# pananananas/MVD

Hardware: AMD Instinct MI355X
Metric: UNet forward-passes/sec @512x512 SD2.1+MV adapter (higher is better)
Workload: dtype bf16; 1 GPU; cfg4: configs[3]/[4]: 8 objects x 4 target views per GPU (32 pairs), camera FiLM + cross-view adapter; pairs_per_gpu=32, global_pairs=32, latent=64x64x4, image=512x512, forward=cold, hip_graph=False, q2_statistics=replica-local, parallelism=dp1 (pairs sharded by object), weights=synthetic seeded, SD2.1 shapes (865.9M UNet x2 + 99.2M adapter + 19.1M camera), encoder_weights=distinct

## Files before the change

### include/mvd_hip.h

```cpp
#ifndef MVD_HIP_H
#define MVD_HIP_H
#include <stddef.h>
#include <stdint.h>

#ifdef __cplusplus
extern "C" {
#endif

#define MVD_MAX_LEVELS 4

typedef struct {
  int in_channels;
  int out_channels;
  int num_levels;
  int block_out_channels[MVD_MAX_LEVELS];
  int num_heads[MVD_MAX_LEVELS];
  int layers_per_block;
  int cross_attention_dim;
  int norm_num_groups;
  float norm_eps;
  int cam_output_dim;
  int cam_hidden_dim;
  int simple_cam_encoder;
  float cam_modulation_strength;
// ... 5 lines not shown

int mvd_engine_create(const mvd_config_t* cfg, mvd_engine_t** out);
int mvd_engine_destroy(mvd_engine_t* e);

int mvd_engine_set_weight(mvd_engine_t* e, int set, const char* slot, const void* ptr, int64_t numel, int dtype);
int mvd_engine_clear_weights(mvd_engine_t* e, int set);

int64_t mvd_engine_workspace_bytes(mvd_engine_t* e, int batch, int height, int width, int text_len, int ref_batch);
int64_t mvd_engine_refcache_bytes(mvd_engine_t* e, int ref_batch, int height, int width, int keep_features);
int mvd_engine_bind_workspace(mvd_engine_t* e, void* ws, int64_t ws_bytes, void* refcache, int64_t refcache_bytes);

enum {
  MVD_USE_CAMERA = 1,
  MVD_USE_IMAGE = 2,
  MVD_REUSE_REF = 4,
  MVD_KEEP_FEATURES = 8
};

typedef struct {
  int batch;
  int height, width;
  int text_len;
  const float* sample;
  const float* timesteps;
  const float* text;
  const float* source_camera;
  const float* target_camera;
  int cam_rows;
  int cam_batch;
  const float* fourier_proj;
  const float* source_latents;
  const float* encoder_text;
  int ref_batch;
  int flags;
  float* out;
} mvd_forward_args_t;

int mvd_unet_forward(mvd_engine_t* e, const mvd_forward_args_t* args, void* stream);

int64_t mvd_engine_reference_pixels(mvd_engine_t* e, int height, int width);
int mvd_engine_reference_encode(mvd_engine_t* e, const mvd_forward_args_t* args, float* local_stats, void* stream);
int mvd_engine_reference_finish(mvd_engine_t* e, const float* mean_k, void* stream);

int mvd_engine_set_graph(mvd_engine_t* e, int enable);

int mvd_engine_share_encoder_weights(mvd_engine_t* e, int enable);

int mvd_engine_set_profiling(mvd_engine_t* e, int enable);
int mvd_engine_profile_summary(mvd_engine_t* e, int cap, int* cls, int* launches, double* ms, double* flops, double* bytes);
int mvd_engine_profile_shapes(mvd_engine_t* e, char* buf_host, int cap);

int mvd_engine_num_features(mvd_engine_t* e);
int mvd_engine_feature_shape(mvd_engine_t* e, int idx, int* channels, int* height, int* width);
// ... 192 lines not shown
```

### mvd_amd/_lib.py

```python
from __future__ import annotations

import ctypes as C
import enum
import os

HERE = os.path.dirname(os.path.abspath(__file__))
LIB_PATH = os.environ.get("MVD_HIP_LIB") or os.path.join(HERE, "libmvd_hip.so")

MVD_MAX_LEVELS = 4
MVD_USE_CAMERA, MVD_USE_IMAGE, MVD_REUSE_REF, MVD_KEEP_FEATURES = 1, 2, 4, 8


class MvdError(RuntimeError):
    pass


class DebugFlag(enum.IntFlag):
    NO_SM_LN_FOLD = 1
    SM_NO_SPLITK = 2
    NO_SM = 4
    NO_SPLIT_KV = 8
    ONE_STREAM = 16
    SINGLE_STREAM_POLICY = 32
    SIDE_DEFAULT_PRIORITY = 64
    NO_XS = 128
# ... 55 lines not shown
        ("fourier_proj", C.c_void_p), ("source_latents", C.c_void_p), ("encoder_text", C.c_void_p),
        ("ref_batch", C.c_int), ("flags", C.c_int), ("out", C.c_void_p),
    ]


_SIGS = {
    "mvd_last_error": (C.c_char_p, []),
    "mvd_engine_create": (C.c_int, [C.POINTER(mvd_config_t), C.POINTER(C.c_void_p)]),
    "mvd_engine_destroy": (C.c_int, [C.c_void_p]),
    "mvd_engine_set_weight": (C.c_int, [C.c_void_p, C.c_int, C.c_char_p, C.c_void_p, C.c_int64, C.c_int]),
    "mvd_engine_clear_weights": (C.c_int, [C.c_void_p, C.c_int]),
    "mvd_engine_workspace_bytes": (C.c_int64, [C.c_void_p, C.c_int, C.c_int, C.c_int, C.c_int, C.c_int]),
    "mvd_engine_refcache_bytes": (C.c_int64, [C.c_void_p, C.c_int, C.c_int, C.c_int, C.c_int]),
    "mvd_engine_bind_workspace": (C.c_int, [C.c_void_p, C.c_void_p, C.c_int64, C.c_void_p, C.c_int64]),
    "mvd_unet_forward": (C.c_int, [C.c_void_p, C.POINTER(mvd_forward_args_t), C.c_void_p]),
    "mvd_engine_set_profiling": (C.c_int, [C.c_void_p, C.c_int]),
    "mvd_engine_profile_summary": (C.c_int, [C.c_void_p, C.c_int, C.POINTER(C.c_int), C.POINTER(C.c_int),
                                             C.POINTER(C.c_double), C.POINTER(C.c_double), C.POINTER(C.c_double)]),
    "mvd_engine_profile_shapes": (C.c_int, [C.c_void_p, C.c_char_p, C.c_int]),
    "mvd_engine_set_graph": (C.c_int, [C.c_void_p, C.c_int]),
    "mvd_engine_reference_pixels": (C.c_int64, [C.c_void_p, C.c_int, C.c_int]),
    "mvd_engine_reference_encode": (C.c_int, [C.c_void_p, C.POINTER(mvd_forward_args_t), C.c_void_p, C.c_void_p]),
    "mvd_engine_reference_finish": (C.c_int, [C.c_void_p, C.c_void_p, C.c_void_p]),
    "mvd_engine_share_encoder_weights": (C.c_int, [C.c_void_p, C.c_int]),
    "mvd_engine_num_features": (C.c_int, [C.c_void_p]),
    "mvd_engine_feature_shape": (C.c_int, [C.c_void_p, C.c_int, C.POINTER(C.c_int), C.POINTER(C.c_int), C.POINTER(C.c_int)]),
    "mvd_engine_get_feature": (C.c_int, [C.c_void_p, C.c_int, C.c_void_p, C.c_void_p]),
    "mvd_engine_encode_cameras": (C.c_int, [C.c_void_p, C.c_void_p, C.c_void_p, C.c_int, C.c_int, C.c_void_p, C.c_void_p, C.c_void_p]),
    "mvd_engine_apply_modulation": (C.c_int, [C.c_void_p, C.c_char_p, C.c_void_p, C.c_int, C.c_void_p, C.c_int, C.c_int, C.c_void_p, C.c_void_p]),
    "mvd_engine_get_camera_embedding": (C.c_int, [C.c_void_p, C.c_void_p, C.c_void_p]),
# ... 140 lines not shown
```

### mvd_amd/csrc/engine.hip

```cpp
#include <math.h>
#include <stdio.h>
#include <stdlib.h>
#include <string.h>

#include <string>
#include <unordered_map>
#include <vector>

#include "host_util.h"

int mvd_launch_silu_to_bf16(const float* x, int64_t n, bf16_t* y, hipStream_t s);

static int g_debug_flags = 0;
extern "C" int mvd_debug_set_flags(int flags) { g_debug_flags = flags; return 0; }
int mvd_debug_flags() { return g_debug_flags; }

namespace {

struct FeatureInfo { std::string name; int level; int C; int heads; std::string key;  };
constexpr int MVD_REF_ONLY_INTERNAL = 1 << 30;

}

struct mvd_engine {
// ... 15 lines not shown
  hipStream_t side = nullptr;
  std::vector<hipEvent_t> feat_ev;
  hipEvent_t fork_ev = nullptr, join_ev = nullptr;
  bool dual_now = false;
  int ensure_side_stream() {
    if (side) return 0;
    {
      int lo = 0, hi = 0;
      (void)hipDeviceGetStreamPriorityRange(&lo, &hi);
      const int pr = (g_debug_flags & MVD_DBG_SIDE_DEFAULT_PRIORITY) ? 0 : hi;
      if (hipStreamCreateWithPriority(&side, hipStreamNonBlocking, pr) != hipSuccess) { mvd_set_error("engine: hipStreamCreate failed"); return -3; }
    }
    feat_ev.resize(feats.size());
    for (auto& ev : feat_ev) if (hipEventCreateWithFlags(&ev, hipEventDisableTiming) != hipSuccess) { mvd_set_error("engine: hipEventCreate failed"); return -3; }
    if (hipEventCreateWithFlags(&fork_ev, hipEventDisableTiming) != hipSuccess || hipEventCreateWithFlags(&join_ev, hipEventDisableTiming) != hipSuccess) { mvd_set_error("engine: hipEventCreate failed"); return -3; }
    return 0;
  }
  bool share_encoder = false;
  struct HostState {
    std::vector<bf16_t*> refkv, feat_keep;
    int rc_batch, rc_h, rc_w; bool rc_valid, rc_keep;
    float* cam_emb; int cam_batch;
  };
  HostState host_state() const { return {refkv, feat_keep, rc_batch, rc_h, rc_w, rc_valid, rc_keep, cam_emb, cam_batch}; }
  void set_host_state(const HostState& h) {
    refkv = h.refkv; feat_keep = h.feat_keep; rc_batch = h.rc_batch; rc_h = h.rc_h; rc_w = h.rc_w; rc_valid = h.rc_valid;
    rc_keep = h.rc_keep; cam_emb = h.cam_emb; cam_batch = h.cam_batch;
  }
  struct GraphEntry { std::string key; hipGraph_t g; hipGraphExec_t x; HostState after; };
  bool dual_late = false;
  bool graph_on = false;
  std::vector<GraphEntry> graphs;
  std::vector<std::string> graph_seen;
  void drop_graphs() {
    for (auto& ge : graphs) { (void)hipGraphExecDestroy(ge.x); (void)hipGraphDestroy(ge.g); }
    graphs.clear(); graph_seen.clear();
  }
  ~mvd_engine() {
    drop_graphs();
    for (hipEvent_t ev : ev_pool) (void)hipEventDestroy(ev);
    for (hipEvent_t ev : feat_ev) if (ev) (void)hipEventDestroy(ev);
    if (fork_ev) (void)hipEventDestroy(fork_ev);
    if (join_ev) (void)hipEventDestroy(join_ev);
    if (side) (void)hipStreamDestroy(side);
  }
  std::vector<int> temb_off;
  int temb_total = 0;
  std::vector<int> tkv_off;
  int tkv_total = 0;
  bool prof = false;
  bool prof_overlap = false;
  struct ProfRec { int cls; double flops; double bytes; hipEvent_t e0, e1; int M, N, K, tag; };
  int prof_M = 0, prof_N = 0, prof_K = 0, prof_tag = 0;
  std::vector<ProfRec> prof_recs;
  std::vector<hipEvent_t> ev_pool; size_t ev_used = 0;
  hipEvent_t get_event() {
// ... 431 lines not shown
      CHECK(c.attention(a));
      CHECK(c.linear(o_self, o_ref, C, ad ? C : 0, M, c.WB(key + ".attn1.out.w", (int64_t)C * ld_out), c.WF(key + ".attn1" + bias_slot, C), C, h, C, h, C, false, false, ld_out,
                     ad ? std::string() : key + ".attn1.out.wx"));
    }
    {
      const int nq = ad ? 2 * C : C;
      bf16_t* q2 = c.talloc<bf16_t>((size_t)M * nq);
      const bf16_t* kv2 = tkv + c.e->tkv_off[feat_idx];
      const int ldkv = c.e->tkv_total;
      CHECK(c.ln_linear(h, M, C, key + ".ln2", key + ".attn2.q", (int64_t)(packed ? 2 : 1) * C, nq, nullptr, ln, q2, nq, false));
      MvdAttnArgs a; memset(&a, 0, sizeof(a));
      a.batch = B_; a.heads = heads; a.scale = scale; a.prescaled = 1; a.nprob = ad ? 2 : 1;
      a.p[0] = {q2, kv2, kv2 + C, o_self, nq, ldkv, ldkv, C, (int64_t)hw * nq, (int64_t)L * ldkv, (int64_t)L * ldkv, (int64_t)hw * C, hw, L};
      if (ad) a.p[1] = {q2 + C, rkv + 2 * C, rkv + 3 * C, o_ref, nq, 4 * C, 4 * C, C, (int64_t)hw * nq, (int64_t)ref_nk * 4 * C, (int64_t)ref_nk * 4 * C, (int64_t)hw * C, hw, ref_nk};
      CHECK(c.attention(a));
      CHECK(c.linear(o_self, o_ref, C, ad ? C : 0, M, c.WB(key + ".attn2.out.w", (int64_t)C * ld_out), c.WF(key + ".attn2" + bias_slot, C), C, h, C, h, C, false, false, ld_out,
                     ad ? std::string() : key + ".attn2.out.wx"));
    }
    {
      bf16_t* ff = c.talloc<bf16_t>((size_t)M * 4 * C);
      CHECK(c.ln_linear(h, M, C, key + ".ln3", key + ".ff1", (int64_t)8 * C, 8 * C, c.WF(key + ".ff1.b", 8 * C), ln, ff, 4 * C, true));
      CHECK(c.linear(ff, nullptr, 4 * C, 0, M, c.WB(key + ".ff2.w", (int64_t)C * 4 * C), c.WF(key + ".ff2.b", C), C, h, C, h, C));
    }
    CHECK(c.linear(h, nullptr, C, 0, M, c.WB(key + ".proj_out.w", (int64_t)C * C), c.WF(key + ".proj_out.b", C), C, x.p, C, out.p, C, false, false, 0, key + ".proj_out.wx"));
    c.e->tmp.off = mark;

    if (o.capture) {
      const size_t mk = c.e->tmp.off;
      bf16_t* rn = c.talloc<bf16_t>((size_t)M * C);
      if (o.defer_norm) {
        if (!c.dry && !c.err) CHECK(mvd_launch_refstats(out.p, B_, hw, C, o.stats + 2 * c.e->feat_pixel_off(feat_idx), c.s));
      } else {
        if (!c.dry && !c.err) CHECK(mvd_launch_refnorm(out.p, B_, hw, C, rn, c.s));
        CHECK(c.linear(rn, nullptr, C, 0, M, c.WB(key + ".ref_kv.w", (int64_t)4 * C * C, 0), nullptr, 4 * C, nullptr, 0, c.e->refkv[feat_idx], 4 * C, false, false, 0,
                       key + ".ref_kv.wx", 0));
        if (c.e->dual_now && !c.dry && !c.err && hipEventRecord(c.e->feat_ev[feat_idx], c.s) != hipSuccess) { mvd_set_error("forward: hipEventRecord failed"); return -3; }
      }
      if (c.e->rc_keep && !c.dry && !c.err)
        CHECK((int)hipMemcpyAsync(c.e->feat_keep[feat_idx], out.p, (size_t)M * C * sizeof(bf16_t), hipMemcpyDeviceToDevice, c.s));
      c.e->tmp.off = mk;
    }
    ++feat_idx;
    return c.err;
  }

  int film(const std::string& name, const Act& x, Act& out) {
    auto it = o.film_ss->find(name);
    if (it == o.film_ss->end()) { out = x; return 0; }
// ... 283 lines not shown
        const int lv = e->feats[i].level;
        const size_t hw = (size_t)(H >> lv) * (Wd >> lv);
        e->refkv[i] = (bf16_t*)e->persist.alloc((size_t)a.ref_batch * hw * 4 * e->feats[i].C * sizeof(bf16_t));
        if (keep) e->feat_keep[i] = (bf16_t*)e->persist.alloc((size_t)a.ref_batch * hw * e->feats[i].C * sizeof(bf16_t));
      }
      if (e->persist.overflow()) { mvd_set_error("forward: reference cache too small (%zu > %zu bytes)", e->persist.high, e->persist.cap); return -4; }
      e->rc_keep = keep; e->rc_batch = a.ref_batch; e->rc_h = H; e->rc_w = Wd;
      if (!dry) { e->rc_valid = false; e->rc_pending = false; }
    }
  }

  const bool dual = use_img && !reuse && !ref_only;
  e->dual_late = false;
  e->dual_now = dual && !dry && !(e->graph_on && (g_debug_flags & MVD_DBG_GRAPH_ONE_STREAM)) && (!e->prof || e->prof_overlap) && !(g_debug_flags & MVD_DBG_ONE_STREAM);
  const bool early = dual && (g_debug_flags & MVD_DBG_FORK_LATE);
  auto fork = [&]() -> int {
    if (!e->dual_now) return 0;
    CHECK(e->ensure_side_stream());
    if (hipEventRecord(e->fork_ev, s) != hipSuccess || hipStreamWaitEvent(e->side, e->fork_ev, 0) != hipSuccess) { mvd_set_error("forward: stream fork failed"); return -3; }
    return 0;
  };
  if (!early) CHECK(fork());

  std::unordered_map<std::string, std::pair<float*, float*>> film_ss;
  if (use_cam) CHECK(camera_path(c, a, film_ss));
  const float* tproj_main = nullptr;
  const float* tproj_enc = nullptr;
  if (early) {
    c.set = 0;
    CHECK(time_path(c, a.timesteps, B, &tproj_main));
    c.set = e->share_encoder ? 0 : 1;
    float* tz = c.aalloc<float>(a.ref_batch);
    if (!dry) CHECK((int)hipMemsetAsync(tz, 0, a.ref_batch * sizeof(float), s));
    CHECK(time_path(c, tz, a.ref_batch, &tproj_enc));
    c.set = 0;
    CHECK(fork());
  }

  if (use_img && !reuse) {
    if (dual) e->tmp.off = e->tmp.high;
    const size_t tm = e->tmp.off, am = e->act.off;
    if (e->dual_now) { c.s = e->side; c.nowait = true; }
    c.set = e->share_encoder ? 0 : 1;
    const int Br = a.ref_batch;
    const float* tproj = tproj_enc;
    if (!tproj) {
      float* tz = c.talloc<float>(Br);
      if (!dry) CHECK((int)hipMemsetAsync(tz, 0, Br * sizeof(float), c.s));
      CHECK(time_path(c, tz, Br, &tproj));
    }
    bf16_t* tx = c.aalloc<bf16_t>((size_t)Br * L * xd);
    Act xin = c.new_act(Br, H, Wd, 64, true);
    if (!dry && !c.err) {
      CHECK(mvd_launch_f32_to_bf16(a.encoder_text, (int64_t)Br * L * xd, tx, c.s));
      CHECK(mvd_launch_im2col_in(a.source_latents, Br, cfg.in_channels, H, Wd, nullptr, nullptr, 0, xin.p, c.s));
    }
    PassOpts po; po.capture = true; po.ref_batch = Br;
    po.defer_norm = ref_only; po.stats = e->ref_stats_out;
    UNetPass pass{c, cfg, po, Br, H, Wd, L, tx, tproj};
    CHECK(pass.run(xin, nullptr));
    if (!dry) { e->rc_valid = !ref_only; e->rc_pending = ref_only; }
    if (dual) {
      e->tmp.off = e->tmp.high;
      if (e->dual_now && hipEventRecord(e->join_ev, e->side) != hipSuccess) { mvd_set_error("forward: hipEventRecord failed"); return -3; }
      c.s = s; c.nowait = false;
    } else {
      e->tmp.off = tm; e->act.off = am;
    }
  }
  if (ref_only) {
    if (c.err) return c.err;
    if (!dry && (e->tmp.high + e->act.high > (size_t)e->ws_bytes)) { mvd_set_error("reference_encode: workspace too small"); return -4; }
    return 0;
  }

  c.set = 0;
  const float* tproj = tproj_main;
  if (!tproj) CHECK(time_path(c, a.timesteps, B, &tproj));
  bf16_t* tx = c.aalloc<bf16_t>((size_t)B * L * xd);
  Act xin = c.new_act(B, H, Wd, 64, true);
  if (!dry && !c.err) {
    CHECK(mvd_launch_f32_to_bf16(a.text, (int64_t)B * L * xd, tx, s));
    const float* sc = nullptr; const float* sh = nullptr;
    if (use_cam) { sc = film_ss["output"].first; sh = film_ss["output"].second; }
    CHECK(mvd_launch_im2col_in(a.sample, B, cfg.in_channels, H, Wd, sc, sh, 4, xin.p, s));
  }
  PassOpts po; po.adapter = use_img; po.film = use_cam; po.ref_batch = a.ref_batch; po.film_ss = &film_ss;
  static const int late_dflt = MVD_ENV_INT("MVD_DUAL_LATE_FROM", 99);
  po.late_from = (g_debug_flags & MVD_DBG_LATE_FROM_UP1) ? 1 : late_dflt;
  UNetPass pass{c, cfg, po, B, H, Wd, L, tx, tproj};
  CHECK(pass.run(xin, a.out));
  if (e->dual_now) {
    if (hipStreamWaitEvent(s, e->join_ev, 0) != hipSuccess) { mvd_set_error("forward: stream join failed"); return -3; }
    e->dual_now = false;
  }
  if (c.err) return c.err;
  if (!dry && (e->tmp.high + e->act.high > (size_t)e->ws_bytes)) { mvd_set_error("forward: workspace too small"); return -4; }
  return 0;
}

int forward_impl(mvd_engine* e, const mvd_forward_args_t& a, hipStream_t s, bool dry) {
  const int r = forward_body(e, a, s, dry);
  if (e->dual_now) {
    if (e->side) (void)hipStreamSynchronize(e->side);
    e->dual_now = false;
  }
  return r;
}

int reference_finish_impl(mvd_engine* e, const float* mean_k, hipStream_t s, bool dry) {
  e->tmp.reset(dry);
  Ctx c{e, s, 0, dry};
  CHECK(setup_tile_counters(e, (unsigned int*)e->tmp.alloc(MVD_TILE_COUNTERS * sizeof(unsigned int)), s, dry));
  c.set = 0;
  for (size_t i = 0; i < e->feats.size(); ++i) {
    const int lv = e->feats[i].level, C = e->feats[i].C;
    const int hw = (e->rc_h >> lv) * (e->rc_w >> lv), M = e->rc_batch * hw;
    const std::string& key = e->feats[i].key;
    const size_t mk = e->tmp.off;
    bf16_t* rn = c.talloc<bf16_t>((size_t)M * C);
    if (!dry && !c.err) CHECK(mvd_launch_refapply(e->feat_keep[i], e->rc_batch, hw, C, mean_k + 2 * e->feat_pixel_off((int)i), rn, s));
// ... 31 lines not shown
  e->cfg = *cfg;
  e->feats = enumerate_features(*cfg);
  int off = 0;
  for (auto& r : enumerate_resnets(*cfg)) { e->temb_off.push_back(off); off += r.cout; }
  e->temb_total = off;
  off = 0;
  for (auto& f : e->feats) { e->tkv_off.push_back(off); off += 2 * f.C; }
  e->tkv_total = off;
  *out = e;
  return 0;
}

int mvd_engine_destroy(mvd_engine_t* e) { delete e; return 0; }

int mvd_engine_set_weight(mvd_engine_t* e, int set, const char* slot, const void* ptr, int64_t numel, int dtype) {
  if (e) e->drop_graphs();
  if (!e || set < 0 || set > 1 || !slot || !ptr || numel <= 0 || dtype < 0 || dtype > 1) { mvd_set_error("set_weight: bad argument"); return -1; }
  if ((uintptr_t)ptr & 15) { mvd_set_error("set_weight: '%s' must be 16-byte aligned", slot); return -1; }
  e->w[set].m[slot] = Weight{ptr, numel, dtype};
  return 0;
}
int mvd_engine_clear_weights(mvd_engine_t* e, int set) {
  if (e) e->drop_graphs();
  if (!e || set < 0 || set > 1) { mvd_set_error("clear_weights: bad argument"); return -1; }
  e->w[set].m.clear();
  return 0;
}

static void fill_dry_args(mvd_forward_args_t& a, int batch, int h, int w, int L, int ref_batch) {
  memset(&a, 0, sizeof(a));
  a.batch = batch; a.height = h; a.width = w; a.text_len = L; a.ref_batch = ref_batch; a.cam_rows = 4;
  a.flags = MVD_USE_CAMERA | (ref_batch > 0 ? MVD_USE_IMAGE : 0);
}

int64_t mvd_engine_workspace_bytes(mvd_engine_t* e, int batch, int height, int width, int text_len, int ref_batch) {
  if (!e) { mvd_set_error("workspace_bytes: null engine"); return -1; }
  mvd_forward_args_t a; fill_dry_args(a, batch, height, width, text_len, ref_batch);
  const mvd_engine::HostState before = e->host_state();
// ... 3 lines not shown
  return (int64_t)(((e->act.high + 255) & ~size_t(255)) + e->tmp.high + 4096);
}

int64_t mvd_engine_refcache_bytes(mvd_engine_t* e, int ref_batch, int height, int width, int keep_features) {
  if (!e || ref_batch <= 0) { mvd_set_error("refcache_bytes: bad argument"); return -1; }
  size_t total = 0;
  for (auto& f : e->feats) {
    const size_t hw = (size_t)(height >> f.level) * (width >> f.level);
    total += (((size_t)ref_batch * hw * 4 * f.C * 2) + 255) & ~size_t(255);
    if (keep_features) total += (((size_t)ref_batch * hw * f.C * 2) + 255) & ~size_t(255);
  }
  return (int64_t)total + 4096;
}

int mvd_engine_bind_workspace(mvd_engine_t* e, void* ws, int64_t ws_bytes, void* refcache, int64_t refcache_bytes) {
  if (e) e->drop_graphs();
  if (!e || !ws || ws_bytes <= 0) { mvd_set_error("bind_workspace: bad argument"); return -1; }
  if (((uintptr_t)ws & 255) || (refcache && ((uintptr_t)refcache & 255))) { mvd_set_error("bind_workspace: buffers must be 256-byte aligned"); return -1; }
  e->ws_ptr = ws; e->ws_bytes = ws_bytes;
  e->rc_ptr = refcache; e->rc_bytes = refcache_bytes;
  e->persist.base = (char*)refcache; e->persist.cap = (size_t)(refcache ? refcache_bytes : 0);
  e->rc_valid = false; e->rc_pending = false;
  return 0;
}

int64_t mvd_engine_reference_pixels(mvd_engine_t* e, int height, int width) {
  if (!e || height <= 0 || width <= 0) { mvd_set_error("reference_pixels: bad argument"); return -1; }
  return e->ref_pixels(height, width);
}

int mvd_engine_reference_encode(mvd_engine_t* e, const mvd_forward_args_t* args, float* local_stats, void* stream) {
  if (!e || !args || !local_stats) { mvd_set_error("reference_encode: null argument"); return -1; }
  e->drop_graphs();
  mvd_forward_args_t a = *args;
  a.flags = (a.flags & ~MVD_REUSE_REF) | MVD_USE_IMAGE | MVD_KEEP_FEATURES | MVD_REF_ONLY_INTERNAL;
  if (a.batch <= 0) a.batch = a.ref_batch;
  int r = forward_impl(e, a, nullptr, true);
  e->rc_valid = false; e->rc_pending = false;
  if (r) return r;
  const size_t act_bytes = (e->act.high + 255) & ~size_t(255);
  if (!e->ws_ptr || act_bytes + e->tmp.high > (size_t)e->ws_bytes) {
    mvd_set_error("reference_encode: workspace too small: need %zu bytes, bound %lld", act_bytes + e->tmp.high, (long long)e->ws_bytes);
    return -4;
  }
  e->act.base = (char*)e->ws_ptr; e->act.cap = act_bytes;
  e->tmp.base = (char*)e->ws_ptr + act_bytes; e->tmp.cap = (size_t)e->ws_bytes - act_bytes;
  e->ref_stats_out = local_stats;
  r = forward_impl(e, a, (hipStream_t)stream, false);
  e->ref_stats_out = nullptr;
  return r;
}

int mvd_engine_reference_finish(mvd_engine_t* e, const float* mean_k, void* stream) {
  if (!e || !mean_k) { mvd_set_error("reference_finish: null argument"); return -1; }
  if (!e->rc_pending) { mvd_set_error("reference_finish: no pending reference (call mvd_engine_reference_encode first)"); return -1; }
  e->drop_graphs();
  int r = reference_finish_impl(e, mean_k, nullptr, true);
  if (r) return r;
  if (!e->ws_ptr || e->tmp.high > (size_t)e->ws_bytes) { mvd_set_error("reference_finish: workspace too small (%zu > %lld bytes)", e->tmp.high, (long long)e->ws_bytes); return -4; }
  e->tmp.base = (char*)e->ws_ptr; e->tmp.cap = (size_t)e->ws_bytes;
  r = reference_finish_impl(e, mean_k, (hipStream_t)stream, false);
  if (r) return r;
  e->rc_pending = false; e->rc_valid = true;
  return 0;
}

int mvd_unet_forward(mvd_engine_t* e, const mvd_forward_args_t* args, void* stream) {
  if (!e || !args) { mvd_set_error("forward: null argument"); return -1; }
  if (args->flags & MVD_REF_ONLY_INTERNAL) { mvd_set_error("forward: unknown flag bits 0x%x", args->flags); return -1; }
  const mvd_engine::HostState before = e->host_state();
  int r = forward_impl(e, *args, nullptr, true);
  e->set_host_state(before);
  if (r) return r;
  const size_t act_bytes = (e->act.high + 255) & ~size_t(255);
  if (!e->ws_ptr || act_bytes + e->tmp.high > (size_t)e->ws_bytes) {
    mvd_set_error("forward: workspace too small: need %zu bytes, bound %lld", act_bytes + e->tmp.high, (long long)e->ws_bytes);
    return -4;
  }
  e->act.base = (char*)e->ws_ptr; e->act.cap = act_bytes;
  e->tmp.base = (char*)e->ws_ptr + act_bytes; e->tmp.cap = (size_t)e->ws_bytes - act_bytes;
  hipStream_t st = (hipStream_t)stream;
  if (!e->graph_on || e->prof || !st) return forward_impl(e, *args, st, false);
  std::string key((const char*)args, sizeof(*args));
  const int st8[8] = {e->rc_valid, e->rc_batch, e->rc_h, e->rc_w, e->rc_keep, e->share_encoder, 0, 0};
  key.append((const char*)st8, sizeof(st8));
  key.append((const char*)&e->ws_ptr, sizeof(void*));
  key.append((const char*)&e->rc_ptr, sizeof(void*));
  for (auto& ge : e->graphs)
    if (ge.key == key) {
      hipError_t he = hipGraphLaunch(ge.x, st);
      if (he != hipSuccess) { mvd_set_error("forward: hipGraphLaunch: %s", hipGetErrorString(he)); return -7; }
      e->set_host_state(ge.after);
      return 0;
    }
  bool seen = false;
  for (auto& k : e->graph_seen) seen |= k == key;
// ... 3 lines not shown
  if (he != hipSuccess) { mvd_set_error("forward: hipStreamBeginCapture: %s", hipGetErrorString(he)); return -7; }
  r = forward_impl(e, *args, st, false);
  hipGraph_t g = nullptr;
  he = hipStreamEndCapture(st, &g);
  if (r) { if (g) (void)hipGraphDestroy(g); return r; }
  if (he != hipSuccess || !g) { mvd_set_error("forward: hipStreamEndCapture: %s", hipGetErrorString(he)); return -7; }
  hipGraphExec_t x = nullptr;
  he = hipGraphInstantiate(&x, g, nullptr, nullptr, 0);
  if (he != hipSuccess) { (void)hipGraphDestroy(g); mvd_set_error("forward: hipGraphInstantiate: %s", hipGetErrorString(he)); return -7; }
  e->graphs.push_back({key, g, x, e->host_state()});
  he = hipGraphLaunch(x, st);
  if (he != hipSuccess) { mvd_set_error("forward: hipGraphLaunch: %s", hipGetErrorString(he)); return -7; }
  return 0;
}

int mvd_engine_set_graph(mvd_engine_t* e, int enable) {
  if (!e) { mvd_set_error("set_graph: null engine"); return -1; }
  e->graph_on = enable != 0;
  if (!e->graph_on) e->drop_graphs();
  return 0;
}

int mvd_engine_set_profiling(mvd_engine_t* e, int enable) {
  if (!e) { mvd_set_error("set_profiling: null engine"); return -1; }
  e->prof = enable != 0; e->prof_overlap = enable == 2; e->prof_recs.clear(); e->ev_used = 0;
  return 0;
}

int mvd_engine_profile_summary(mvd_engine_t* e, int cap, int* cls, int* launches, double* ms, double* flops, double* bytes) {
  if (!e || cap <= 0 || !cls || !launches || !ms || !flops || !bytes) { mvd_set_error("profile_summary: bad argument"); return -1; }
  int n = 0;
  for (auto& r : e->prof_recs) {
    if (hipEventSynchronize(r.e1) != hipSuccess) { mvd_set_error("profile_summary: event sync failed"); return -2; }
    float t = 0.f;
    if (hipEventElapsedTime(&t, r.e0, r.e1) != hipSuccess) { mvd_set_error("profile_summary: elapsed time failed"); return -2; }
    int j = 0;
    while (j < n && cls[j] != r.cls) ++j;
    if (j == n) { if (n == cap) continue; cls[n] = r.cls; launches[n] = 0; ms[n] = 0; flops[n] = 0; bytes[n] = 0; ++n; }
    launches[j] += 1; ms[j] += t; flops[j] += r.flops; bytes[j] += r.bytes;
// ... 13 lines not shown
    while (j < v.size() && !(v[j].cls == r.cls && v[j].M == r.M && v[j].N == r.N && v[j].K == r.K && v[j].tag == r.tag)) ++j;
    if (j == v.size()) v.push_back({r.cls, r.M, r.N, r.K, r.tag, 0, 0.0, 0.0});
    v[j].n++; v[j].ms += t; v[j].fl += r.flops;
  }
  int off = 0;
  for (auto& x : v) {
    const int w = snprintf(buf + off, (size_t)(cap - off), "cls=%d M=%d N=%d K=%d tag=%d launches=%d ms=%.3f tflops=%.0f\n", x.cls, x.M, x.N, x.K,
                           x.tag, x.n, x.ms, x.ms > 0 ? x.fl / x.ms / 1e9 : 0.0);
    if (w < 0 || off + w >= cap) break;
    off += w;
  }
  return off;
}

int mvd_engine_share_encoder_weights(mvd_engine_t* e, int enable) {
  if (e) e->drop_graphs();
  if (!e) { mvd_set_error("share_encoder_weights: null engine"); return -1; }
  e->share_encoder = enable != 0;
  return 0;
}

int mvd_engine_num_features(mvd_engine_t* e) { return e ? (int)e->feats.size() : -1; }
int mvd_engine_feature_shape(mvd_engine_t* e, int idx, int* channels, int* height, int* width) {
  if (!e || idx < 0 || idx >= (int)e->feats.size() || !e->rc_h) { mvd_set_error("feature_shape: bad index or no reference pass yet"); return -1; }
  *channels = e->feats[idx].C; *height = e->rc_h >> e->feats[idx].level; *width = e->rc_w >> e->feats[idx].level;
  return 0;
}
int mvd_engine_get_feature(mvd_engine_t* e, int idx, float* out_nchw, void* stream) {
  if (!e || idx < 0 || idx >= (int)e->feats.size() || !out_nchw) { mvd_set_error("get_feature: bad argument"); return -1; }
  if (!e->rc_valid || !e->rc_keep || !e->feat_keep[idx]) { mvd_set_error("get_feature: no kept features (run forward with MVD_KEEP_FEATURES)"); return -1; }
  const int lv = e->feats[idx].level;
  return mvd_launch_nhwc_to_nchw_f32(e->feat_keep[idx], e->rc_batch, (e->rc_h >> lv) * (e->rc_w >> lv), e->feats[idx].C, out_nchw, (hipStream_t)stream);
}
int mvd_engine_encode_cameras(mvd_engine_t* e, const float* source_camera, const float* target_camera, int cam_rows,
                              int batch, const float* fourier_proj, float* out_emb, void* stream) {
  if (!e || !source_camera || !target_camera || !fourier_proj || !out_emb || batch <= 0 || (cam_rows != 3 && cam_rows != 4)) { mvd_set_error("encode_cameras: bad argument"); return -1; }
  if (!e->ws_ptr) { mvd_set_error("encode_cameras: workspace not bound"); return -1; }
  {
    e->tmp.reset(true);
    Ctx d{e, nullptr, 0, true};
    if (int r = camera_embed(d, source_camera, target_camera, cam_rows, fourier_proj, batch, out_emb)) return r;
    if (e->tmp.high > (size_t)e->ws_bytes) { mvd_set_error("encode_cameras: workspace too small (%zu > %lld bytes)", e->tmp.high, (long long)e->ws_bytes); return -4; }
  }
  e->tmp.reset(false); e->tmp.base = (char*)e->ws_ptr; e->tmp.cap = (size_t)e->ws_bytes;
  Ctx c{e, (hipStream_t)stream, 0, false};
  return camera_embed(c, source_camera, target_camera, cam_rows, fourier_proj, batch, out_emb);
}

int mvd_engine_apply_modulation(mvd_engine_t* e, const char* name, const float* emb, int batch, const float* x_nchw,
                                int channels, int hw, float* out_nchw, void* stream) {
  if (!e || !name || !emb || !x_nchw || !out_nchw || batch <= 0 || channels <= 0 || hw <= 0) { mvd_set_error("apply_modulation: bad argument"); return -1; }
  if (!e->ws_ptr) { mvd_set_error("apply_modulation: workspace not bound"); return -1; }
  int dim = -1;
  for (auto& m : modulator_dims(e->cfg, true)) if (m.first == name) dim = m.second;
  if (dim < 0) return 1;
  if (dim != channels) { mvd_set_error("apply_modulation: modulator '%s' has %d channels, tensor has %d", name, dim, channels); return -1; }
  {
    e->tmp.reset(true);
    Ctx d{e, nullptr, 0, true};
    float* sc0 = d.talloc<float>((size_t)batch * dim);
    float* sh0 = d.talloc<float>((size_t)batch * dim);
    if (int r = modulator(d, name, dim, emb, batch, sc0, sh0)) return r;
    if (e->tmp.high > (size_t)e->ws_bytes) { mvd_set_error("apply_modulation: workspace too small (%zu > %lld bytes)", e->tmp.high, (long long)e->ws_bytes); return -4; }
  }
  e->tmp.reset(false); e->tmp.base = (char*)e->ws_ptr; e->tmp.cap = (size_t)e->ws_bytes;
  Ctx c{e, (hipStream_t)stream, 0, false};
  float* sc = c.talloc<float>((size_t)batch * dim);
// ... 133 lines not shown
```

### mvd_amd/engine.py

```python
from __future__ import annotations

import ctypes as C
import os
from typing import Dict, List, Optional

import torch

from . import _lib as L
from .config import UNetConfig
from .packing import pack_camera, pack_unet


def _ptr(t: Optional[torch.Tensor]):
    return None if t is None else C.c_void_p(t.data_ptr())


def _stream():
    return C.c_void_p(torch.cuda.current_stream().cuda_stream)


class MVDEngine:
    def __init__(self, cfg: UNetConfig, cam_output_dim: int = 1024, cam_hidden_dim: int = 512,
                 simple_cam_encoder: bool = False, cam_modulation_strength: float = 0.2, device="cuda:0",
                 small_batch_twins: Optional[bool] = None):
# ... 94 lines not shown
        if self._ws is None or self._ws.numel() < ws:
            self._ws = None
            self._ws = torch.empty(ws, dtype=torch.uint8, device=self.device)
        if rc and (self._rc is None or self._rc.numel() < rc):
            self._rc = None
            self._rc = torch.empty(rc, dtype=torch.uint8, device=self.device)
        L.call("mvd_engine_bind_workspace", self._h, _ptr(self._ws), self._ws.numel(),
               _ptr(self._rc) if rc else None, self._rc.numel() if rc else 0)
        self._ws_key = key
        self._ref_valid = None

    def forward(self, sample: torch.Tensor, timesteps: torch.Tensor, text: torch.Tensor,
                source_camera: Optional[torch.Tensor] = None, target_camera: Optional[torch.Tensor] = None,
                fourier_proj: Optional[torch.Tensor] = None, source_latents: Optional[torch.Tensor] = None,
                encoder_text: Optional[torch.Tensor] = None, reuse_ref: bool = False,
                keep_features: bool = False, out: Optional[torch.Tensor] = None) -> torch.Tensor:
        B, Cin, H, W = sample.shape
        Lt = text.shape[1]
        for t in (sample, timesteps, text, source_camera, target_camera, fourier_proj, source_latents, encoder_text):
            if t is not None:
                if not (t.is_cuda and t.dtype == torch.float32 and t.is_contiguous()):
                    raise L.MvdError("engine.forward expects contiguous fp32 CUDA tensors")
        if text.shape[0] != B or timesteps.shape != (B,):
            raise L.MvdError(f"engine.forward: text batch {text.shape[0]} / timesteps {tuple(timesteps.shape)} vs batch {B}")
        use_cam = target_camera is not None
        use_img = source_latents is not None or reuse_ref
        ref_batch = 0
        if use_img:
            ref_batch = source_latents.shape[0] if source_latents is not None else self._last_ref_batch
            self._last_ref_batch = ref_batch
        self._ensure_workspace(B, H, W, Lt, ref_batch, keep_features)
# ... 22 lines not shown
            a.source_camera, a.target_camera = source_camera.data_ptr(), target_camera.data_ptr()
            a.cam_rows = source_camera.shape[1]
            a.cam_batch = Bc
            a.fourier_proj = fourier_proj.data_ptr()
            flags |= L.MVD_USE_CAMERA
        if use_img:
            flags |= L.MVD_USE_IMAGE
            if reuse_ref:
                flags |= L.MVD_REUSE_REF
            else:
                if encoder_text is None or encoder_text.shape[0] != ref_batch:
                    raise L.MvdError("image conditioning needs encoder_text with the reference batch")
                a.source_latents, a.encoder_text = source_latents.data_ptr(), encoder_text.data_ptr()
            if keep_features:
                flags |= L.MVD_KEEP_FEATURES
        a.ref_batch, a.flags = ref_batch, flags
        a.out = out.data_ptr()
        if graph:
            cur = torch.cuda.current_stream(self.device)
            self._gstream.wait_stream(cur)
            with torch.cuda.stream(self._gstream):
                L.call("mvd_unet_forward", self._h, C.byref(a), _stream())
            cur.wait_stream(self._gstream)
            out = out.clone() if user_out is None else user_out.copy_(out)
        else:
            L.call("mvd_unet_forward", self._h, C.byref(a), _stream())
        if use_img and not reuse_ref:
            self._ref_valid = (B, H, W, Lt, ref_batch)
        return out

# ... 24 lines not shown
            n[off:off + h_.value * w_.value] = float(Br * c_.value)
            off += h_.value * w_.value
        return torch.cat([n[:, None], stats], dim=1)

    def reference_finish(self, mean_k: torch.Tensor) -> None:
        pend = getattr(self, "_ref_pending", None)
        if pend is None:
            raise L.MvdError("reference_finish without a pending reference_encode")
        npix = L.lib().mvd_engine_reference_pixels(self._h, pend[1], pend[2])
        if not (mean_k.is_cuda and mean_k.dtype == torch.float32 and mean_k.is_contiguous() and tuple(mean_k.shape) == (npix, 2)):
            raise L.MvdError(f"reference_finish expects a contiguous fp32 CUDA tensor [{npix}, 2]")
        L.call("mvd_engine_reference_finish", self._h, _ptr(mean_k), _stream())
        self._ref_pending = None
        self._ref_valid = pend

    def set_graph(self, enable: bool) -> None:
        L.call("mvd_engine_set_graph", self._h, int(bool(enable)))
        self._graph = bool(enable)
        if enable and getattr(self, "_gstream", None) is None:
            self._gstream = torch.cuda.Stream(device=self.device)
            self._gbufs = {}

    def _staged(self, name: str, t: torch.Tensor, shape=None) -> torch.Tensor:
        shape = tuple(t.shape) if shape is None else tuple(shape)
        buf = self._gbufs.get((name, shape))
        if buf is None:
            buf = self._gbufs[(name, shape)] = torch.empty(shape, dtype=torch.float32, device=self.device)
        if name != "out":
            buf.copy_(t)
        return buf
# ... 49 lines not shown
```

### mvd_amd/mvd_unet.py

```python
from __future__ import annotations

import logging
import os
from typing import Any, Dict, NamedTuple, Optional

import torch
import torch.nn as nn

from . import _lib as L
from .attention import get_attention_processor_for_module
from .camera_encoder import CameraEncoder
from .config import UNetConfig
from .unet_params import UNet2DConditionParams

logger = logging.getLogger(__name__)


class UNetOutput(NamedTuple):
    sample: torch.FloatTensor


def _build_unet(cfg: UNetConfig, init: str) -> UNet2DConditionParams:
    if init == "empty":
        with torch.device("meta"):
# ... 116 lines not shown
            self.camera_encoder = None
        if use_image_conditioning:
            self.image_encoder = ImageEncoder(snapshot, dtype=dtype,
                                              expected_sample_size=self.config.sample_size, unet_config=cfg, init=init)
            self.image_encoder._encode_fn = self._encode_reference
        else:
            self.image_encoder = None
        self.hooks = []
        self._init_image_cross_attention()
        self.to(dtype=dtype)

        self._engine = None
        self._dirty = True
        self._ref_key = None
        self._ref_hold = None
        self.reference_stats_group = None
        self.current_camera_embedding = None
        self.fourier_projection = None

    def _init_image_cross_attention(self):
        self.attention_layer_map = {}
        self.feature_to_attention_map = {}
        with torch.no_grad():
            for key, feat, _c, _h in self.unet_config.transformers():
                tb = self.base_unet.get_submodule(key).transformer_blocks[0]
                for attn, suffix in ((tb.attn1, "_self"), (tb.attn2, "_cross")):
                    name = feat + suffix
                    proc = get_attention_processor_for_module(name, attn, img_ref_scale=self.img_ref_scale)
                    self.attention_layer_map[name] = attn
                    attn.processor = proc
# ... 44 lines not shown
            self.encoder_weights_shared = False
            if self.image_encoder is not None:
                esd = self.image_encoder.unet.state_dict()
                share = self.dedup_encoder_weights
                if share == "auto":
                    share = all(k in sd and sd[k].shape == v.shape and torch.equal(sd[k], v.to(sd[k].device)) for k, v in esd.items())
                if share:
                    self._engine.share_encoder_weights(True)
                    self.encoder_weights_shared = True
                else:
                    self._engine.load_image_encoder(esd)
            self._dirty = False
            self.reset_reference_cache()
        if bool(getattr(self, "use_hip_graph", False)) != bool(getattr(self._engine, "_graph", False)):
            self._engine.set_graph(bool(getattr(self, "use_hip_graph", False)))
        return self._engine

    def reset_reference_cache(self):
        self._ref_key = None
        self._ref_hold = None

    @staticmethod
    def _f32(t: torch.Tensor, dev) -> torch.Tensor:
        return t.to(device=dev, dtype=torch.float32).contiguous()

    def _encode_reference(self, latents, text) -> Dict[str, torch.Tensor]:
        eng = self._sync_engine()
        dev = eng.device
        lat, txt = self._f32(latents, dev), self._f32(text, dev)
        B = lat.shape[0]
        dummy_t = torch.zeros(B, device=dev, dtype=torch.float32)
        eng.forward(lat, dummy_t, txt, source_latents=lat, encoder_text=txt, keep_features=True)
        self.reset_reference_cache()
        return eng.features()

# ... 30 lines not shown
            if text.shape[0] == 2 * bs:
                enc_text = text[bs:]
            elif text.shape[0] > bs:
                enc_text = text[:bs]
            key = (source_image_latents.data_ptr(), source_image_latents._version, tuple(source_image_latents.shape),
                   encoder_hidden_states.data_ptr(), encoder_hidden_states._version, tuple(encoder_hidden_states.shape), B)
            glob = self.reference_stats_group is not None
            hit = (self.cache_reference and self._ref_key == key
                   and eng.reference_cache_valid(B, x.shape[2], x.shape[3], text.shape[1], bs))
            if glob and self.cache_reference:
                from .distributed import any_rank
                hit = not any_rank(not hit, None if self.reference_stats_group is True else self.reference_stats_group, dev)
            if hit:
                img = dict(reuse_ref=True, keep_features=glob)
            else:
                img = dict(source_latents=self._f32(source_image_latents, dev), encoder_text=enc_text.contiguous())
                self._ref_key = key
                self._ref_hold = (source_image_latents, encoder_hidden_states) if self.cache_reference else None
                if glob:
                    from .distributed import merge_reference_stats
                    group = None if self.reference_stats_group is True else self.reference_stats_group
                    local = eng.reference_encode(img["source_latents"], img["encoder_text"], B)
                    eng.reference_finish(merge_reference_stats(local, group))
                    img = dict(reuse_ref=True, keep_features=True)
        out = eng.forward(x, t, text, **cam, **img)
        if cam:
            self.current_camera_embedding = eng.camera_embedding(cam["target_camera"].shape[0])
        hidden_states = out.to(out_dtype)
        if not return_dict:
            return hidden_states
        return UNetOutput(sample=hidden_states)

    def _map_image_features_to_attention_layers(self, image_features):
# ... 23 lines not shown
```

Before: 543.5 forward-passes/s.

## Start next forward's reference encoder early, overlapping the previous forward's tail

When the reference inputs (source latents and encoder text) are unchanged from the previous call and the workspace layout matches, the side-stream encoder pass skips the fork wait on the main stream. It can therefore begin while the previous forward's decoder is still running. Per-feature 'consumed' events are recorded after each ref-attention read, and the encoder waits on them before overwriting the matching ref KV buffer. The encoder also gets its own tile-counter region. On the Python side the f32-converted reference tensors are kept and reused across calls, so the device pointers stay stable. The price is a lot of state validation (arena marks, weight epoch, stream, pointers) and a risk of cross-call hazards if any invariant is missed.

```diff
diff --git a/include/mvd_hip.h b/include/mvd_hip.h
--- a/include/mvd_hip.h
+++ b/include/mvd_hip.h
@@ -43,7 +43,8 @@
   MVD_USE_CAMERA = 1,
   MVD_USE_IMAGE = 2,
   MVD_REUSE_REF = 4,
-  MVD_KEEP_FEATURES = 8
+  MVD_KEEP_FEATURES = 8,
+  MVD_REF_INPUTS_UNCHANGED = 16
 };
 
 typedef struct {
@@ -66,6 +67,9 @@
 } mvd_forward_args_t;
 
 int mvd_unet_forward(mvd_engine_t* e, const mvd_forward_args_t* args, void* stream);
+
+int mvd_engine_set_forward_overlap(mvd_engine_t* e, int enable);
+int mvd_engine_last_forward_overlapped(mvd_engine_t* e);
 
 int64_t mvd_engine_reference_pixels(mvd_engine_t* e, int height, int width);
 int mvd_engine_reference_encode(mvd_engine_t* e, const mvd_forward_args_t* args, float* local_stats, void* stream);
diff --git a/mvd_amd/_lib.py b/mvd_amd/_lib.py
--- a/mvd_amd/_lib.py
+++ b/mvd_amd/_lib.py
@@ -8,7 +8,7 @@
 LIB_PATH = os.environ.get("MVD_HIP_LIB") or os.path.join(HERE, "libmvd_hip.so")
 
 MVD_MAX_LEVELS = 4
-MVD_USE_CAMERA, MVD_USE_IMAGE, MVD_REUSE_REF, MVD_KEEP_FEATURES = 1, 2, 4, 8
+MVD_USE_CAMERA, MVD_USE_IMAGE, MVD_REUSE_REF, MVD_KEEP_FEATURES, MVD_REF_INPUTS_UNCHANGED = 1, 2, 4, 8, 16
 
 
 class MvdError(RuntimeError):
@@ -94,6 +94,8 @@
     "mvd_engine_refcache_bytes": (C.c_int64, [C.c_void_p, C.c_int, C.c_int, C.c_int, C.c_int]),
     "mvd_engine_bind_workspace": (C.c_int, [C.c_void_p, C.c_void_p, C.c_int64, C.c_void_p, C.c_int64]),
     "mvd_unet_forward": (C.c_int, [C.c_void_p, C.POINTER(mvd_forward_args_t), C.c_void_p]),
+    "mvd_engine_set_forward_overlap": (C.c_int, [C.c_void_p, C.c_int]),
+    "mvd_engine_last_forward_overlapped": (C.c_int, [C.c_void_p]),
     "mvd_engine_set_profiling": (C.c_int, [C.c_void_p, C.c_int]),
     "mvd_engine_profile_summary": (C.c_int, [C.c_void_p, C.c_int, C.POINTER(C.c_int), C.POINTER(C.c_int),
                                              C.POINTER(C.c_double), C.POINTER(C.c_double), C.POINTER(C.c_double)]),
diff --git a/mvd_amd/csrc/engine.hip b/mvd_amd/csrc/engine.hip
--- a/mvd_amd/csrc/engine.hip
+++ b/mvd_amd/csrc/engine.hip
@@ -53,8 +53,30 @@
     feat_ev.resize(feats.size());
     for (auto& ev : feat_ev) if (hipEventCreateWithFlags(&ev, hipEventDisableTiming) != hipSuccess) { mvd_set_error("engine: hipEventCreate failed"); return -3; }
     if (hipEventCreateWithFlags(&fork_ev, hipEventDisableTiming) != hipSuccess || hipEventCreateWithFlags(&join_ev, hipEventDisableTiming) != hipSuccess) { mvd_set_error("engine: hipEventCreate failed"); return -3; }
+    consumed_ev.resize(feats.size());
+    for (auto& ev : consumed_ev) if (hipEventCreateWithFlags(&ev, hipEventDisableTiming) != hipSuccess) { mvd_set_error("engine: hipEventCreate failed"); return -3; }
     return 0;
   }
+  std::vector<hipEvent_t> consumed_ev;
+  struct EncMarks { size_t tmp_lo = 0, tmp_hi = 0, act_lo = 0, act_hi = 0; };
+  struct OverlapState {
+    bool ok = false;
+    const void* src = nullptr; const void* txt = nullptr;
+    int ref_batch = 0, h = 0, w = 0, text_len = 0;
+    const char* act_base = nullptr; const char* tmp_base = nullptr; const void* rc_ptr = nullptr; int64_t ws_bytes = 0, rc_bytes = 0;
+    EncMarks marks;
+    unsigned long long weight_epoch = 0;
+    hipStream_t stream = nullptr;
+  };
+  OverlapState prev;
+  bool prev_live = false;
+  EncMarks enc_marks;
+  unsigned long long weight_epoch = 0;
+  bool overlap_on = true;
+  bool early_now = false;
+  bool track_consumed = false;
+  bool last_early = false;
+  void overlap_break() { prev.ok = false; prev_live = false; }
   bool share_encoder = false;
   struct HostState {
     std::vector<bf16_t*> refkv, feat_keep;
@@ -79,6 +101,7 @@
     drop_graphs();
     for (hipEvent_t ev : ev_pool) (void)hipEventDestroy(ev);
     for (hipEvent_t ev : feat_ev) if (ev) (void)hipEventDestroy(ev);
+    for (hipEvent_t ev : consumed_ev) if (ev) (void)hipEventDestroy(ev);
     if (fork_ev) (void)hipEventDestroy(fork_ev);
     if (join_ev) (void)hipEventDestroy(join_ev);
     if (side) (void)hipStreamDestroy(side);
@@ -540,6 +563,7 @@
       a.p[0] = {q2, kv2, kv2 + C, o_self, nq, ldkv, ldkv, C, (int64_t)hw * nq, (int64_t)L * ldkv, (int64_t)L * ldkv, (int64_t)hw * C, hw, L};
       if (ad) a.p[1] = {q2 + C, rkv + 2 * C, rkv + 3 * C, o_ref, nq, 4 * C, 4 * C, C, (int64_t)hw * nq, (int64_t)ref_nk * 4 * C, (int64_t)ref_nk * 4 * C, (int64_t)hw * C, hw, ref_nk};
       CHECK(c.attention(a));
+      if (ad && c.e->track_consumed && !c.dry && !c.err && hipEventRecord(c.e->consumed_ev[feat_idx], c.s) != hipSuccess) { mvd_set_error("forward: hipEventRecord failed"); return -3; }
       CHECK(c.linear(o_self, o_ref, C, ad ? C : 0, M, c.WB(key + ".attn2.out.w", (int64_t)C * ld_out), c.WF(key + ".attn2" + bias_slot, C), C, h, C, h, C, false, false, ld_out,
                      ad ? std::string() : key + ".attn2.out.wx"));
     }
@@ -558,6 +582,7 @@
         if (!c.dry && !c.err) CHECK(mvd_launch_refstats(out.p, B_, hw, C, o.stats + 2 * c.e->feat_pixel_off(feat_idx), c.s));
       } else {
         if (!c.dry && !c.err) CHECK(mvd_launch_refnorm(out.p, B_, hw, C, rn, c.s));
+        if (c.e->early_now && !c.dry && !c.err && hipStreamWaitEvent(c.s, c.e->consumed_ev[feat_idx], 0) != hipSuccess) { mvd_set_error("forward: hipStreamWaitEvent failed"); return -3; }
         CHECK(c.linear(rn, nullptr, C, 0, M, c.WB(key + ".ref_kv.w", (int64_t)4 * C * C, 0), nullptr, 4 * C, nullptr, 0, c.e->refkv[feat_idx], 4 * C, false, false, 0,
                        key + ".ref_kv.wx", 0));
         if (c.e->dual_now && !c.dry && !c.err && hipEventRecord(c.e->feat_ev[feat_idx], c.s) != hipSuccess) { mvd_set_error("forward: hipEventRecord failed"); return -3; }
@@ -871,9 +896,23 @@
   e->dual_late = false;
   e->dual_now = dual && !dry && !(e->graph_on && (g_debug_flags & MVD_DBG_GRAPH_ONE_STREAM)) && (!e->prof || e->prof_overlap) && !(g_debug_flags & MVD_DBG_ONE_STREAM);
   const bool early = dual && (g_debug_flags & MVD_DBG_FORK_LATE);
+  const bool plain = e->dual_now && !early && e->overlap_on && !e->graph_on && !e->prof && !(a.flags & MVD_KEEP_FEATURES);
+  e->track_consumed = plain;
+  e->early_now = false;
+  if (plain && (a.flags & MVD_REF_INPUTS_UNCHANGED) && e->prev_live && e->side) {
+    const mvd_engine::OverlapState& p = e->prev;
+    const mvd_engine::EncMarks& m = e->enc_marks;
+    e->early_now = p.src == a.source_latents && p.txt == a.encoder_text && p.ref_batch == a.ref_batch && p.h == H && p.w == Wd && p.text_len == L &&
+                   p.act_base == e->act.base && p.tmp_base == e->tmp.base && p.ws_bytes == e->ws_bytes && p.rc_ptr == e->rc_ptr && p.rc_bytes == e->rc_bytes &&
+                   p.weight_epoch == e->weight_epoch && p.stream == s &&
+                   p.marks.tmp_lo == m.tmp_lo && p.marks.tmp_hi == m.tmp_hi && p.marks.act_lo == m.act_lo && p.marks.act_hi == m.act_hi &&
+                   m.tmp_lo < m.tmp_hi && m.act_lo < m.act_hi;
+  }
+  if (!dry) { e->prev_live = false; e->last_early = e->early_now; }
   auto fork = [&]() -> int {
     if (!e->dual_now) return 0;
     CHECK(e->ensure_side_stream());
+    if (e->early_now) return 0;
     if (hipEventRecord(e->fork_ev, s) != hipSuccess || hipStreamWaitEvent(e->side, e->fork_ev, 0) != hipSuccess) { mvd_set_error("forward: stream fork failed"); return -3; }
     return 0;
   };
@@ -898,6 +937,8 @@
     if (dual) e->tmp.off = e->tmp.high;
     const size_t tm = e->tmp.off, am = e->act.off;
     if (e->dual_now) { c.s = e->side; c.nowait = true; }
+    unsigned int* const cnt_main = e->cnt_base; const int cnt_main_used = e->cnt_used;
+    if (dual) CHECK(setup_tile_counters(e, (unsigned int*)e->act.alloc(MVD_TILE_COUNTERS * sizeof(unsigned int)), c.s, dry));
     c.set = e->share_encoder ? 0 : 1;
     const int Br = a.ref_batch;
     const float* tproj = tproj_enc;
@@ -919,6 +960,12 @@
     if (!dry) { e->rc_valid = !ref_only; e->rc_pending = ref_only; }
     if (dual) {
       e->tmp.off = e->tmp.high;
+      e->cnt_base = cnt_main; e->cnt_used = cnt_main_used;
+      const mvd_engine::EncMarks m{tm, e->tmp.high, am, e->act.off};
+      if (e->early_now && (m.tmp_lo != e->enc_marks.tmp_lo || m.tmp_hi != e->enc_marks.tmp_hi || m.act_lo != e->enc_marks.act_lo || m.act_hi != e->enc_marks.act_hi)) {
+        mvd_set_error("forward: the encoder pass's arena regions differ from the sizing run's"); return -16;
+      }
+      e->enc_marks = m;
       if (e->dual_now && hipEventRecord(e->join_ev, e->side) != hipSuccess) { mvd_set_error("forward: hipEventRecord failed"); return -3; }
       c.s = s; c.nowait = false;
     } else {
@@ -947,12 +994,20 @@
   po.late_from = (g_debug_flags & MVD_DBG_LATE_FROM_UP1) ? 1 : late_dflt;
   UNetPass pass{c, cfg, po, B, H, Wd, L, tx, tproj};
   CHECK(pass.run(xin, a.out));
+  const bool tracked = e->track_consumed;
+  e->track_consumed = false;
   if (e->dual_now) {
     if (hipStreamWaitEvent(s, e->join_ev, 0) != hipSuccess) { mvd_set_error("forward: stream join failed"); return -3; }
     e->dual_now = false;
   }
   if (c.err) return c.err;
   if (!dry && (e->tmp.high + e->act.high > (size_t)e->ws_bytes)) { mvd_set_error("forward: workspace too small"); return -4; }
+  if (tracked) {
+    mvd_engine::OverlapState& p = e->prev;
+    p.ok = true; p.src = a.source_latents; p.txt = a.encoder_text; p.ref_batch = a.ref_batch; p.h = H; p.w = Wd; p.text_len = L;
+    p.act_base = e->act.base; p.tmp_base = e->tmp.base; p.ws_bytes = e->ws_bytes; p.rc_ptr = e->rc_ptr; p.rc_bytes = e->rc_bytes;
+    p.marks = e->enc_marks; p.weight_epoch = e->weight_epoch; p.stream = s;
+  }
   return 0;
 }
 
@@ -962,6 +1017,7 @@
     if (e->side) (void)hipStreamSynchronize(e->side);
     e->dual_now = false;
   }
+  e->track_consumed = false; e->early_now = false;
   return r;
 }
 
@@ -1023,14 +1079,14 @@
 int mvd_engine_destroy(mvd_engine_t* e) { delete e; return 0; }
 
 int mvd_engine_set_weight(mvd_engine_t* e, int set, const char* slot, const void* ptr, int64_t numel, int dtype) {
-  if (e) e->drop_graphs();
+  if (e) { e->drop_graphs(); ++e->weight_epoch; }
   if (!e || set < 0 || set > 1 || !slot || !ptr || numel <= 0 || dtype < 0 || dtype > 1) { mvd_set_error("set_weight: bad argument"); return -1; }
   if ((uintptr_t)ptr & 15) { mvd_set_error("set_weight: '%s' must be 16-byte aligned", slot); return -1; }
   e->w[set].m[slot] = Weight{ptr, numel, dtype};
   return 0;
 }
 int mvd_engine_clear_weights(mvd_engine_t* e, int set) {
-  if (e) e->drop_graphs();
+  if (e) { e->drop_graphs(); ++e->weight_epoch; }
   if (!e || set < 0 || set > 1) { mvd_set_error("clear_weights: bad argument"); return -1; }
   e->w[set].m.clear();
   return 0;
@@ -1064,7 +1120,7 @@
 }
 
 int mvd_engine_bind_workspace(mvd_engine_t* e, void* ws, int64_t ws_bytes, void* refcache, int64_t refcache_bytes) {
-  if (e) e->drop_graphs();
+  if (e) { e->drop_graphs(); e->overlap_break(); }
   if (!e || !ws || ws_bytes <= 0) { mvd_set_error("bind_workspace: bad argument"); return -1; }
   if (((uintptr_t)ws & 255) || (refcache && ((uintptr_t)refcache & 255))) { mvd_set_error("bind_workspace: buffers must be 256-byte aligned"); return -1; }
   e->ws_ptr = ws; e->ws_bytes = ws_bytes;
@@ -1081,7 +1137,7 @@
 
 int mvd_engine_reference_encode(mvd_engine_t* e, const mvd_forward_args_t* args, float* local_stats, void* stream) {
   if (!e || !args || !local_stats) { mvd_set_error("reference_encode: null argument"); return -1; }
-  e->drop_graphs();
+  e->drop_graphs(); e->overlap_break();
   mvd_forward_args_t a = *args;
   a.flags = (a.flags & ~MVD_REUSE_REF) | MVD_USE_IMAGE | MVD_KEEP_FEATURES | MVD_REF_ONLY_INTERNAL;
   if (a.batch <= 0) a.batch = a.ref_batch;
@@ -1104,7 +1160,7 @@
 int mvd_engine_reference_finish(mvd_engine_t* e, const float* mean_k, void* stream) {
   if (!e || !mean_k) { mvd_set_error("reference_finish: null argument"); return -1; }
   if (!e->rc_pending) { mvd_set_error("reference_finish: no pending reference (call mvd_engine_reference_encode first)"); return -1; }
-  e->drop_graphs();
+  e->drop_graphs(); e->overlap_break();
   int r = reference_finish_impl(e, mean_k, nullptr, true);
   if (r) return r;
   if (!e->ws_ptr || e->tmp.high > (size_t)e->ws_bytes) { mvd_set_error("reference_finish: workspace too small (%zu > %lld bytes)", e->tmp.high, (long long)e->ws_bytes); return -4; }
@@ -1118,6 +1174,8 @@
 int mvd_unet_forward(mvd_engine_t* e, const mvd_forward_args_t* args, void* stream) {
   if (!e || !args) { mvd_set_error("forward: null argument"); return -1; }
   if (args->flags & MVD_REF_ONLY_INTERNAL) { mvd_set_error("forward: unknown flag bits 0x%x", args->flags); return -1; }
+  const bool prev_ok = e->prev.ok;
+  e->overlap_break(); e->last_early = false;
   const mvd_engine::HostState before = e->host_state();
   int r = forward_impl(e, *args, nullptr, true);
   e->set_host_state(before);
@@ -1130,6 +1188,7 @@
   e->act.base = (char*)e->ws_ptr; e->act.cap = act_bytes;
   e->tmp.base = (char*)e->ws_ptr + act_bytes; e->tmp.cap = (size_t)e->ws_bytes - act_bytes;
   hipStream_t st = (hipStream_t)stream;
+  e->prev_live = prev_ok;
   if (!e->graph_on || e->prof || !st) return forward_impl(e, *args, st, false);
   std::string key((const char*)args, sizeof(*args));
   const int st8[8] = {e->rc_valid, e->rc_batch, e->rc_h, e->rc_w, e->rc_keep, e->share_encoder, 0, 0};
@@ -1163,8 +1222,17 @@
   return 0;
 }
 
+int mvd_engine_set_forward_overlap(mvd_engine_t* e, int enable) {
+  if (!e) { mvd_set_error("set_forward_overlap: null engine"); return -1; }
+  e->overlap_on = enable != 0;
+  e->overlap_break();
+  return 0;
+}
+int mvd_engine_last_forward_overlapped(mvd_engine_t* e) { return e ? (e->last_early ? 1 : 0) : -1; }
+
 int mvd_engine_set_graph(mvd_engine_t* e, int enable) {
   if (!e) { mvd_set_error("set_graph: null engine"); return -1; }
+  e->overlap_break();
   e->graph_on = enable != 0;
   if (!e->graph_on) e->drop_graphs();
   return 0;
@@ -1172,6 +1240,7 @@
 
 int mvd_engine_set_profiling(mvd_engine_t* e, int enable) {
   if (!e) { mvd_set_error("set_profiling: null engine"); return -1; }
+  e->overlap_break();
   e->prof = enable != 0; e->prof_overlap = enable == 2; e->prof_recs.clear(); e->ev_used = 0;
   return 0;
 }
@@ -1215,7 +1284,7 @@
 }
 
 int mvd_engine_share_encoder_weights(mvd_engine_t* e, int enable) {
-  if (e) e->drop_graphs();
+  if (e) { e->drop_graphs(); ++e->weight_epoch; }
   if (!e) { mvd_set_error("share_encoder_weights: null engine"); return -1; }
   e->share_encoder = enable != 0;
   return 0;
@@ -1237,6 +1306,7 @@
                               int batch, const float* fourier_proj, float* out_emb, void* stream) {
   if (!e || !source_camera || !target_camera || !fourier_proj || !out_emb || batch <= 0 || (cam_rows != 3 && cam_rows != 4)) { mvd_set_error("encode_cameras: bad argument"); return -1; }
   if (!e->ws_ptr) { mvd_set_error("encode_cameras: workspace not bound"); return -1; }
+  e->overlap_break();
   {
     e->tmp.reset(true);
     Ctx d{e, nullptr, 0, true};
@@ -1252,6 +1322,7 @@
                                 int channels, int hw, float* out_nchw, void* stream) {
   if (!e || !name || !emb || !x_nchw || !out_nchw || batch <= 0 || channels <= 0 || hw <= 0) { mvd_set_error("apply_modulation: bad argument"); return -1; }
   if (!e->ws_ptr) { mvd_set_error("apply_modulation: workspace not bound"); return -1; }
+  e->overlap_break();
   int dim = -1;
   for (auto& m : modulator_dims(e->cfg, true)) if (m.first == name) dim = m.second;
   if (dim < 0) return 1;
diff --git a/mvd_amd/engine.py b/mvd_amd/engine.py
--- a/mvd_amd/engine.py
+++ b/mvd_amd/engine.py
@@ -132,7 +132,8 @@
                 source_camera: Optional[torch.Tensor] = None, target_camera: Optional[torch.Tensor] = None,
                 fourier_proj: Optional[torch.Tensor] = None, source_latents: Optional[torch.Tensor] = None,
                 encoder_text: Optional[torch.Tensor] = None, reuse_ref: bool = False,
-                keep_features: bool = False, out: Optional[torch.Tensor] = None) -> torch.Tensor:
+                keep_features: bool = False, out: Optional[torch.Tensor] = None,
+                ref_inputs_unchanged: bool = False) -> torch.Tensor:
         B, Cin, H, W = sample.shape
         Lt = text.shape[1]
         for t in (sample, timesteps, text, source_camera, target_camera, fourier_proj, source_latents, encoder_text):
@@ -185,6 +186,8 @@
                 a.source_latents, a.encoder_text = source_latents.data_ptr(), encoder_text.data_ptr()
             if keep_features:
                 flags |= L.MVD_KEEP_FEATURES
+            if ref_inputs_unchanged and not reuse_ref and not graph:
+                flags |= L.MVD_REF_INPUTS_UNCHANGED
         a.ref_batch, a.flags = ref_batch, flags
         a.out = out.data_ptr()
         if graph:
@@ -239,6 +242,13 @@
         self._ref_pending = None
         self._ref_valid = pend
 
+    def set_forward_overlap(self, enable: bool) -> None:
+        L.call("mvd_engine_set_forward_overlap", self._h, int(bool(enable)))
+        self._overlap = bool(enable)
+
+    def last_forward_overlapped(self) -> bool:
+        return L.lib().mvd_engine_last_forward_overlapped(self._h) == 1
+
     def set_graph(self, enable: bool) -> None:
         L.call("mvd_engine_set_graph", self._h, int(bool(enable)))
         self._graph = bool(enable)
diff --git a/mvd_amd/mvd_unet.py b/mvd_amd/mvd_unet.py
--- a/mvd_amd/mvd_unet.py
+++ b/mvd_amd/mvd_unet.py
@@ -154,6 +154,8 @@
         self._dirty = True
         self._ref_key = None
         self._ref_hold = None
+        self._ref_sent = None
+        self.overlap_forwards = os.environ.get("MVD_FORWARD_OVERLAP", "1") != "0"
         self.reference_stats_group = None
         self.current_camera_embedding = None
         self.fourier_projection = None
@@ -228,11 +230,14 @@
             self.reset_reference_cache()
         if bool(getattr(self, "use_hip_graph", False)) != bool(getattr(self._engine, "_graph", False)):
             self._engine.set_graph(bool(getattr(self, "use_hip_graph", False)))
+        if bool(getattr(self, "overlap_forwards", True)) != bool(getattr(self._engine, "_overlap", True)):
+            self._engine.set_forward_overlap(bool(getattr(self, "overlap_forwards", True)))
         return self._engine
 
     def reset_reference_cache(self):
         self._ref_key = None
         self._ref_hold = None
+        self._ref_sent = None
 
     @staticmethod
     def _f32(t: torch.Tensor, dev) -> torch.Tensor:
@@ -293,9 +298,13 @@
             if hit:
                 img = dict(reuse_ref=True, keep_features=glob)
             else:
-                img = dict(source_latents=self._f32(source_image_latents, dev), encoder_text=enc_text.contiguous())
+                if self.overlap_forwards and not glob and self._ref_key == key and self._ref_sent is not None:
+                    img = dict(source_latents=self._ref_sent[0], encoder_text=self._ref_sent[1], ref_inputs_unchanged=True)
+                else:
+                    img = dict(source_latents=self._f32(source_image_latents, dev), encoder_text=enc_text.contiguous())
+                    self._ref_sent = (img["source_latents"], img["encoder_text"])
                 self._ref_key = key
-                self._ref_hold = (source_image_latents, encoder_hidden_states) if self.cache_reference else None
+                self._ref_hold = (source_image_latents, encoder_hidden_states)
                 if glob:
                     from .distributed import merge_reference_stats
                     group = None if self.reference_stats_group is True else self.reference_stats_group
```

After: 546.2 forward-passes/s (median of 6 runs). About the same (+0.5%).
